# NikolaZubic/2dimageto3dmodel

Hardware: NVIDIA H100
Metric: render+loss+GAN images/sec (cfg3: cfg2 render+loss at batch 32 + conv-GAN 256x256 G/D iteration, 1 G : 2 D, Adam) (higher is better)
Workload: dtype tf32 (convs) / f32

## Files before the change

2dimageto3dmodel_b200/b3d/conv.py:

```python
import ctypes

import torch

from . import B3DError, check, dev, last_variant, lib, ptr, stream_ptr
from .bank import LayerWeights

VARIANT_LOG = None


def _conv_call(fn, *args):
    rc = fn(*args)
    if VARIANT_LOG is not None and rc == 0:
        VARIANT_LOG.extend(v for v in last_variant().split(";") if v)
    return rc


def _ints(v):
    return (ctypes.c_int * len(v))(*v)


def _pad_last(t, mult):
    c = t.shape[-1]
    return t if c % mult == 0 else torch.nn.functional.pad(t, (0, mult - c % mult))

# ... 204 lines not shown
        N, H, W, _ = x.shape
        gy = dev(gy, "grad_output")
        st = stream_ptr(gy)
        gb = None
        want_gb = has_bias and ctx.needs_input_grad[2]
        g_pitch = 0
        link_out = ctx.link_out
        if link_out is not None and link_out.done:
            link_out.done = False
            if tuple(gy.shape) != tuple(y.shape):
                raise B3DError("conv2d: chained gradient has the wrong shape")
            g_pitch = y.shape[2]
            gb = link_out.gb if want_gb else None
            link_out.gb = None
            gy = gy[:, :, pad_out:y.shape[2] - pad_out]
        elif pad_out:
            _, Ho, OW, _ = y.shape
            masked = torch.empty(N, Ho, OW - 2 * pad_out, Cout, device=gy.device, dtype=torch.float32)
            gb = torch.zeros(Cout, device=gy.device, dtype=torch.float32) if want_gb else None
            check(lib.b3d_pad_leaky_bias_bwd(ptr(gy), ptr(y), ptr(masked), ptr(gb), N * Ho, OW - 2 * pad_out, Cout, pad_out,
                                             pad_mode, float(leaky), st))
            gy = masked
        elif leaky != 1.0:
            masked = torch.empty_like(gy)
            check(lib.b3d_leaky_bwd(ptr(gy), ptr(y), ptr(masked), gy.numel(), float(leaky), st))
            gy = masked
        if gb is None and want_gb:
            gb = gy.sum(dim=(0, 1, 2))
        gx = gw = None
        if ctx.needs_input_grad[0]:
            link_in = ctx.link_in
            sums = torch.zeros(2 * Cin, device=gy.device, dtype=torch.float64) if link_in is not None and link_in.want_gb else None
            gx = _dgrad(gy, lw.wd if lw.wd is not None else _d_layout(lw.wf.detach()), (gy.shape[1] if fold_raw else H, W), kh,
                        kw, pad_y, stride, x_crop, g_pitch, x if link_in is not None else None,
                        link_in.slope if link_in is not None else 1.0, sums)
            if link_in is not None:
                check(lib.b3d_wrap_x_bwd_inplace(ptr(gx), N * H, W - 2 * link_in.pad, Cin, link_in.pad, link_in.mode, st))
                link_in.gb = sums[:Cin].float() if sums is not None else None
                link_in.done = True
            if fold_raw:
                graw = torch.empty(N, H, W, Cx, device=gy.device, dtype=torch.float32)
                check(lib.b3d_fold_rows_bwd(ptr(gx), ptr(graw), N, H, W, Cx, lw.kh, fold_pad, Cin, st))
                gx = graw
            elif Cx != Cin:
                gx = gx[..., :Cx]
        if ctx.needs_input_grad[1]:
            if fold_raw:
                gw = _wgrad(gy, x, kh, kw, fold_pad, stride, x_crop, lw.df, g_pitch, fold_raw, Cin)
            else:
                gw = _wgrad(gy, x, kh, kw, pad_y, stride, x_crop, lw.df, g_pitch)
            if lw.df is None:
                gw = gw[:, :lw.Cin]
        return gx, gw, gb, None, None, None, None, None, None, None, None, None, None, None, None


def fold_kh_weight(weight, cpad=0):
    Cout, Cin, kh, kw = weight.shape
    w = weight.permute(0, 2, 1, 3).reshape(Cout, kh * Cin, 1, kw)
    return torch.nn.functional.pad(w, (0, 0, 0, 0, 0, cpad)) if cpad else w


def conv2d(x_nchw, weight, bias=None, pad_y=0, stride=1, leaky=1.0, pad_out=0, pad_mode=1, x_crop=0):
    x = x_nchw.permute(0, 2, 3, 1)
    Cout, Cin, kh, kw = weight.shape
    if stride == 1 and kh > 1 and Cin * kh <= 64:
        from .ew import fold_rows
        cpad = (-kh * Cin) % 32
        x = fold_rows(x, kh, pad_y, kh * Cin + cpad)
        weight = fold_kh_weight(weight, cpad)
        Cout, Cin, kh, kw = weight.shape
        pad_y = 0
    lw = LayerWeights(dict(Cout=Cout, Cin=Cin, kh=kh, kw=kw, fold=0, Cinp=-(-Cin // 32) * 32, Coutp=-(-Cout // 32) * 32,
                           Tp=kh * kw))
    lw.wf = _pad_last(taps_layout(weight.detach()), 32)
    y = _Conv.apply(x, weight, bias, lw, int(pad_y), int(stride), float(leaky), int(pad_out), int(pad_mode), int(x_crop))
    return y.permute(0, 3, 1, 2)


def conv2d_banked(x_nchw, lw, pad_y=0, stride=1, leaky=1.0, pad_out=0, pad_mode=1, x_crop=0, stats=None, link_in=None, link_out=None):
    x = x_nchw.permute(0, 2, 3, 1)
    fold_raw, fold_fwd = 0, False
    if lw.fold:
        Wout = x.shape[2] - lw.kw + 1
        if (lw.Cin == 8 and lw.kw == 5 and lw.Cinp == 64 and stride == 1 and not x_crop and Wout % 128 == 0
                and x.shape[0] * x.shape[1] * (Wout // 128) >= 2 * torch.cuda.get_device_properties(x.device).multi_processor_count):
            fold_raw = lw.kh
            fold_fwd = torch.is_grad_enabled() and lw.wf.requires_grad
        else:
            from .ew import fold_rows
            x = fold_rows(x, lw.kh, pad_y, lw.Cinp)
    y = _Conv.apply(x, lw.wf, lw.bias, lw, int(pad_y), int(stride), float(leaky), int(pad_out), int(pad_mode), int(x_crop), stats,
                    fold_raw, link_in, link_out, fold_fwd)
    return y.permute(0, 3, 1, 2)
```

2dimageto3dmodel_b200/csrc/b3d_core.cu:

```cuda
#include <atomic>
#include <stdarg.h>
#include <string.h>

#include "b3d_common.cuh"

namespace b3d {
static thread_local char g_err[512] = "";
static thread_local char g_variant[256] = "";
static std::atomic<uint64_t> g_launches{0};

void set_error(const char* fmt, ...) {
    va_list ap;
    va_start(ap, fmt);
    vsnprintf(g_err, sizeof(g_err), fmt, ap);
    va_end(ap);
}
void clear_variant() { g_variant[0] = 0; }
void add_variant(const char* fmt, ...) {
    size_t n = strlen(g_variant);
    if (n + 2 >= sizeof(g_variant)) return;
    if (n) g_variant[n++] = ';';
    va_list ap;
    va_start(ap, fmt);
    vsnprintf(g_variant + n, sizeof(g_variant) - n, fmt, ap);
    va_end(ap);
}
void count_launch(int n) { g_launches.fetch_add((uint64_t)n, std::memory_order_relaxed); }
}

extern "C" {
const char* b3d_last_error(void) { return b3d::g_err; }
const char* b3d_last_variant(void) { return b3d::g_variant; }
int b3d_version(void) { return 420; }
uint64_t b3d_launch_count(void) { return b3d::g_launches.load(std::memory_order_relaxed); }
}
```

2dimageto3dmodel_b200/csrc/tc_conv.cu:

```cuda
#include "tc_common.cuh"

namespace {

constexpr int BM = 128;
constexpr int BK = 32;
constexpr int MMA_K = 8;
constexpr int MAX_TAPS = 25;
constexpr int NTHREADS = 384;

struct ConvParams {
    int N, Hout, Wout, Cout;
    int BW, BH, BI;
    int tiles_x, tiles_y;
    int xbase;
    int ntaps, kslices;
    int sy, sx;
    int dy[MAX_TAPS], dx[MAX_TAPS];
    int wtap[MAX_TAPS];
    int OH, OW, OC, osy, osx;
    float leaky;
    double* stats;
    int fold;
    int fold_y0;
    int mask;
    float mslope;
    int stats_sum;
    int ncls;
    int cooy[4], coox[4];
    uint32_t esn, esy, esx;
    int dx0, shift[5];
};

constexpr int MASK_BYTES = BM * BK * 4;
template <int BN, int STAGES, int KW>
struct CSmem {
    static constexpr int WIN_BYTES = (BM + KW - 1) * BK * 4;
    static constexpr int A_BYTES = (WIN_BYTES + 1023) / 1024 * 1024;
    static constexpr int B_BYTES = KW * BN * BK * 4;
    static constexpr int STAGE_BYTES = A_BYTES + B_BYTES;
    static constexpr int TX_BYTES = WIN_BYTES + B_BYTES;
    static constexpr int TOTAL = STAGES * STAGE_BYTES + 1024  + 256 ;
    static_assert(A_BYTES >= MASK_BYTES, "a mask chunk does not fit the A region of a stage");
};

__device__ __forceinline__ uint32_t mask_offset(int px, int ch) { return px * 128 + ((((ch >> 2) ^ px) & 7) << 4) + (ch & 3) * 4; }

template <int BN>
constexpr bool kCoop = BN > 128;
template <int BN>
constexpr int kBlocks = (kCoop<BN> ? BN / 2 : BN) / 64;
template <int BN>
constexpr int kEmptyArrivals = kCoop<BN> ? 8 : 4;
template <int BN>
constexpr int kLeaderArrivals = kEmptyArrivals<BN> / (kCoop<BN> ? 2 : 1);
static_assert(kLeaderArrivals<64> == 4 && kLeaderArrivals<128> == 4 && kLeaderArrivals<256> == 4,
              "a leader stands for the 4 warps of its warpgroup");
template <int BN>
constexpr int kMaskGroup = kCoop<BN> ? 4 : 2;
__host__ __device__ constexpr int mask_chunk_channel(int i, int G) { return 128 * ((i % G) / 2) + 64 * (i / G) + 32 * (i % 2); }

template <int BN, int STAGES, int KW, bool FOLD>
__device__ __forceinline__ void mainloop(float (&acc)[kBlocks<BN>][BM / 2], unsigned char* base, uint64_t* full, uint64_t* empty,
                                         int KI, uint32_t& git, uint32_t& phase, int cb, bool leader, const int* shift) {
    constexpr int A_BYTES = CSmem<BN, STAGES, KW>::A_BYTES, STAGE = CSmem<BN, STAGES, KW>::STAGE_BYTES;
    for (int it = 0; it < KI; ++it, ++git) {
        const int s = git % STAGES;
        tc::mbar_wait(full + s, (phase >> s) & 1);
        phase ^= 1u << s;
        const uint32_t a = tc::smem_u32(base + s * STAGE), b = a + A_BYTES + cb * 128;
        tc::wgmma_fence();
#pragma unroll
        for (int t = 0; t < KW; ++t) {
            const uint32_t shifted = a + (KW > 1 ? shift[t] * 128 : 0);
#pragma unroll
            for (int k = 0; k < BK / MMA_K; ++k) {
                const uint32_t acc_flag = (it | t | k) ? 1u : 0u;
                const uint64_t dp = FOLD ? tc::desc_k32(a + k * (BM * 32)) : tc::desc_k128(shifted + k * MMA_K * 4);
#pragma unroll
                for (int m = 0; m < kBlocks<BN>; ++m)
                    tc::Wgmma<BM>::mma(acc[m], tc::desc_k128(b + t * (BN * 128) + m * (64 * 128) + k * MMA_K * 4), dp, acc_flag);
            }
        }
        tc::wgmma_commit();
        tc::wgmma_wait<1>();
        if (it > 0 && leader) tc::mbar_arrive(empty + (git - 1) % STAGES, kLeaderArrivals<BN>);
    }
    tc::wgmma_wait<0>();
    if (KI > 0 && leader) tc::mbar_arrive(empty + (git - 1) % STAGES, kLeaderArrivals<BN>);
}

struct TileAt {
    int n0, y0, x0;
    size_t base;
    int lbw, lbwh;
};
__device__ __forceinline__ void tile_origin(const ConvParams& p, TileAt& t, int tile, int cls) {
    t.x0 = p.xbase + (tile % p.tiles_x) * p.BW;
    t.y0 = (tile / p.tiles_x) % p.tiles_y * p.BH;
    t.n0 = tile / (p.tiles_x * p.tiles_y) * p.BI;
    t.base = (((size_t)t.n0 * p.OH + (size_t)(p.osy * t.y0 + p.cooy[cls])) * p.OW + (size_t)(p.osx * t.x0 + p.coox[cls])) * p.OC;
}
__device__ __forceinline__ bool tile_pixel(const ConvParams& p, const TileAt& t, int px, uint32_t& rel) {
    const int bi = px >> t.lbwh, by = (px >> t.lbw) & (p.BH - 1), bx = px & (p.BW - 1);
    rel = bi * p.esn + by * p.esy + bx * p.esx;
    return t.n0 + bi < p.N && t.y0 + by < p.Hout && t.x0 + bx < p.Wout;
}

template <int G, int STAGES>
__device__ __forceinline__ void mask_bits(uint32_t (&neg)[2], uint32_t mstage, int cw, int lane, uint64_t* empty, uint32_t g0) {
    int q;
    asm volatile("mov.u32 %0, 0;" : "=r"(q));
    q += 2 * (lane & 3);
    uint32_t mb[4];
#pragma unroll
    for (int i = 0; i < 4; ++i) mb[i] = mstage + mask_offset(q + (i & 1), (cw + 8 * (i >> 1)) & 31);
#pragma unroll
    for (int hf = 0; hf < 2; ++hf) {
        uint32_t bits = 0;
#pragma unroll
        for (int j = 0; j < BM / 16; ++j)
#pragma unroll
            for (int i = 0; i < 4; ++i) bits |= (tc::lds_f32(mb[i] + 1024 * (j + 8 * hf)) >= 0.f ? 0u : 1u) << (4 * j + i);
        neg[hf] = bits;
    }
    __syncwarp();
    if (lane == 0)
#pragma unroll
        for (int i = 0; i < G; ++i) tc::mbar_arrive(empty + (g0 + i) % STAGES);
}

template <bool MASKED>
__device__ __forceinline__ void epilogue_block(const float (&acc)[BM / 2], const uint32_t (&neg)[2], const ConvParams& p, const TileAt& t,
                                               const float* bias, float* out, int c0, int cw, int lane) {
    bool cok[2];
    float bv[2], sum[2] = {0.f, 0.f}, sq[2] = {0.f, 0.f};
#pragma unroll
    for (int e = 0; e < 2; ++e) {
        cok[e] = c0 + cw + 8 * e < p.Cout;
        bv[e] = bias && cok[e] ? __ldg(bias + c0 + cw + 8 * e) : 0.f;
    }
    float* out0 = out + t.base + c0 + cw;
    int q;
    asm volatile("mov.u32 %0, 0;" : "=r"(q));
    q += 2 * (lane & 3);
#pragma unroll
    for (int j = 0; j < BM / 8; ++j) {
#pragma unroll
        for (int e1 = 0; e1 < 2; ++e1) {
            uint32_t rel;
            const bool valid = tile_pixel(p, t, 8 * j + q + e1, rel);
#pragma unroll
            for (int e2 = 0; e2 < 2; ++e2) {
                float v = acc[4 * j + 2 * e2 + e1];
                if constexpr (MASKED) v *= (neg[j / 8] >> (4 * (j % 8) + 2 * e2 + e1)) & 1u ? p.mslope : 1.f;
                v = valid ? v : 0.f;
                sum[e2] += v;
                sq[e2] += v * v;
                if (valid && cok[e2]) {
                    const float o = v + bv[e2];
                    out0[rel + 8 * e2] = o >= 0.f ? o : o * p.leaky;
                }
            }
        }
    }
    if (p.stats) {
#pragma unroll
        for (int e = 0; e < 2; ++e) {
            sum[e] += __shfl_xor_sync(0xffffffffu, sum[e], 1);
            sum[e] += __shfl_xor_sync(0xffffffffu, sum[e], 2);
            sq[e] += __shfl_xor_sync(0xffffffffu, sq[e], 1);
            sq[e] += __shfl_xor_sync(0xffffffffu, sq[e], 2);
            if ((lane & 3) == 0 && cok[e]) {
                atomicAdd(p.stats + c0 + cw + 8 * e, (double)sum[e]);
                if (!p.stats_sum) atomicAdd(p.stats + p.Cout + c0 + cw + 8 * e, (double)sq[e]);
            }
        }
    }
}

constexpr int PRODUCER_REGS = 24, CONSUMER_REGS = 240;

template <int BN, int STAGES, int KW>
__global__ void __launch_bounds__(NTHREADS, 1)
conv_wgmma_kernel(const __grid_constant__ CUtensorMap tmap_x, const __grid_constant__ CUtensorMap tmap_w,
                  const __grid_constant__ CUtensorMap tmap_m, const ConvParams p, const float* __restrict__ bias,
                  float* __restrict__ out, int tiles, int work_items) {
    using S = CSmem<BN, STAGES, KW>;
    constexpr bool COOP = kCoop<BN>;
    constexpr int OWNERS = COOP ? 1 : 2;
    constexpr int G = kMaskGroup<BN>;
    static_assert(G <= STAGES, "the mask stages of one block do not fit the ring");
    extern __shared__ unsigned char smem_raw[];
    unsigned char* base = reinterpret_cast<unsigned char*>((reinterpret_cast<uintptr_t>(smem_raw) + 1023) & ~uintptr_t(1023));
    uint64_t* full = reinterpret_cast<uint64_t*>(base + STAGES * S::STAGE_BYTES);
    uint64_t* empty = full + OWNERS * STAGES;
    static_assert((OWNERS + 1) * STAGES * 8 <= 256, "barriers do not fit their area");
    if (threadIdx.x == 0) {
        tc::tma_prefetch_desc(&tmap_x);
        tc::tma_prefetch_desc(&tmap_w);
        if (p.mask) tc::tma_prefetch_desc(&tmap_m);
        for (int s = 0; s < STAGES; ++s) {
            for (int o = 0; o < OWNERS; ++o) tc::mbar_init(full + o * STAGES + s, 1);
            tc::mbar_init(empty + s, kEmptyArrivals<BN>);
        }
        tc::fence_barrier_init();
    }
    __syncthreads();
    const int KI = p.ntaps / KW * p.kslices;
    const int MS = p.mask ? BN / 32 : 0;
    const int wg = threadIdx.x >> 7;

    if (wg == 0) {
        tc::setmaxnreg_dec<PRODUCER_REGS>();
        if (threadIdx.x == 0) {
            uint32_t git = 0;
            for (int w = blockIdx.x, k = 0; w < work_items; w += gridDim.x, ++k) {
                uint64_t* fb = full + (COOP ? 0 : (k & 1) * STAGES);
                const int cls = w % p.ncls, wq = w / p.ncls, tb = cls * p.ntaps;
                int t = wq % tiles;
                const int c0 = (wq / tiles) * BN;
                const int x0 = p.xbase + (t % p.tiles_x) * p.BW;
                t /= p.tiles_x;
                const int y0 = (t % p.tiles_y) * p.BH, n0 = (t / p.tiles_y) * p.BI;
                for (int it = 0; it < KI; ++it, ++git) {
                    const int s = git % STAGES;
                    tc::mbar_wait(empty + s, ((git / STAGES) & 1) ^ 1);
                    const int tap = it / p.kslices * KW, ks = it % p.kslices;
                    unsigned char* a = base + s * S::STAGE_BYTES;
                    tc::mbar_arrive_expect_tx(fb + s, S::TX_BYTES);
                    if (KW > 1)
                        tc::tma_load_4d(a, &tmap_x, fb + s, ks * BK, x0 + p.dx0, y0 + p.dy[tb + tap], n0);
                    else if (p.fold)
                        tc::tma_load_4d(a, &tmap_x, fb + s, 0, x0 + p.dx[tb + tap], y0 + p.fold_y0 + 4 * ks, n0);
                    else
                        tc::tma_load_4d(a, &tmap_x, fb + s, ks * BK, p.sx * x0 + p.dx[tb + tap], p.sy * y0 + p.dy[tb + tap], n0);
                    tc::tma_load_3d(a + S::A_BYTES, &tmap_w, fb + s, ks * BK, c0, p.wtap[tb + tap]);
                }
                const int mx = p.osx * x0 + p.coox[cls], my = p.osy * y0 + p.cooy[cls];
                for (int m = 0; m < MS; ++m, ++git) {
                    const int s = git % STAGES;
                    tc::mbar_wait(empty + s, ((git / STAGES) & 1) ^ 1);
                    tc::mbar_arrive_expect_tx(fb + s, MASK_BYTES);
                    tc::tma_load_4d(base + s * S::STAGE_BYTES, &tmap_m, fb + s, c0 + mask_chunk_channel(m, G), mx, my, n0);
                }
            }
        }
        return;
    }
    tc::setmaxnreg_inc<CONSUMER_REGS>();

    const int h = wg - 1, tid = threadIdx.x & 127, lane = tid & 31;
    float acc[kBlocks<BN>][BM / 2];
#pragma unroll
    for (int m = 0; m < kBlocks<BN>; ++m)
#pragma unroll
        for (int i = 0; i < BM / 2; ++i) acc[m][i] = 0.f;
    uint32_t git = 0, phase = 0;
    const uint32_t ring = tc::smem_u32(base);
    TileAt at;
    at.lbw = __ffs(p.BW) - 1;
    at.lbwh = at.lbw + __ffs(p.BH) - 1;
    uint64_t* fb = full + (COOP ? 0 : h * STAGES);
    const int cb = COOP ? 128 * h : 0;
    const int cw = (tid >> 5) * 16 + (lane >> 2);
    const int mine = (COOP ? 2 * h : 0) + (tid >> 6);
    for (int k = COOP ? 0 : h;; k += COOP ? 1 : 2) {
        const int w = blockIdx.x + k * gridDim.x;
        if (w >= work_items) break;
        git = (uint32_t)k * (KI + MS);
        const int wq = w / p.ncls, tile = wq % tiles, c0 = (wq / tiles) * BN + cb;
        tile_origin(p, at, tile, w % p.ncls);
        if (KW == 1 && p.fold) mainloop<BN, STAGES, KW, true>(acc, base, fb, empty, KI, git, phase, cb, tid == 0, p.shift);
        else mainloop<BN, STAGES, KW, false>(acc, base, fb, empty, KI, git, phase, cb, tid == 0, p.shift);
        uint32_t neg[kBlocks<BN>][2] = {};
        if (p.mask) {
#pragma unroll
            for (int m = 0; m < kBlocks<BN>; ++m, git += G) {
                uint32_t mstage = 0;
#pragma unroll
                for (int i = 0; i < G; ++i) {
                    const int s = (git + i) % STAGES;
                    tc::mbar_wait(fb + s, (phase >> s) & 1);
                    phase ^= 1u << s;
                    if (i == mine) mstage = ring + s * S::STAGE_BYTES;
                }
                mask_bits<G, STAGES>(neg[m], mstage, cw, lane, empty, git);
            }
        }
#pragma unroll
        for (int m = 0; m < kBlocks<BN>; ++m) {
            if (p.mask) epilogue_block<true>(acc[m], neg[m], p, at, bias, out, c0 + 64 * m, cw, lane);
            else epilogue_block<false>(acc[m], neg[m], p, at, bias, out, c0 + 64 * m, cw, lane);
        }
    }
}

struct WgradParams {
    int N, Hout, Wout, Cout, Cin;
    int BWk, BHk;
    int kx, ky;
    int kh, kw, pad_y, st;
    int xoff;
    int splits;
    int tapmajor;
    int tstep;
};

template <int BN, int STAGES, int NRAW, int T>
struct WSmem {
    static constexpr int DY_BYTES = BM * BK * 4;
    static constexpr int STAGE_BYTES = T * BN * BK * 4;
    static constexpr int WROWS = T == 1 ? 32 : 36;
    static constexpr int RAW_X = (BN / 32) * WROWS * 128;
    static constexpr int RAW_BYTES = (DY_BYTES + RAW_X + 1023) / 1024 * 1024;
    static constexpr int TOTAL = STAGES * STAGE_BYTES + NRAW * RAW_BYTES + 1024 + 256;
};

__host__ __device__ constexpr int wgrad_row_co(int m) { return (m & 35) | ((m & 8) >> 1) | ((m & 16) >> 1) | ((m & 4) << 2); }

__host__ __device__ constexpr int dy_tile_offset(int co, int px) {
    return (co >> 5) * 4096 + px * 128 + ((((co >> 2) & 7) ^ (px & 7)) << 4) + (co & 3) * 4;
}

__host__ __device__ constexpr int xt_chunk(int i) { return (((i & 7) >> 1) ^ ((i >> 4) & 3)) | (((i >> 3) & 1) << 2); }
__host__ __device__ constexpr int xt_src_offset(int i, int px, int wrows) { return ((i >> 6) * wrows + px) * 128 + (i & 7) * 16; }
__host__ __device__ constexpr int xt_dst_offset(int i, int j) {
    return ((i >> 6) * 32 + 4 * (i & 7) + j) * 128 + ((xt_chunk(i) ^ ((4 * (i & 7) + j) & 7)) << 4);
}
template <int BN, int T, int WROWS>
__device__ __forceinline__ void wgrad_transpose(uint32_t src, uint32_t dst, int tid) {
    constexpr int NT = 2 * BN / 128;
    float4 v[NT][T + 3];
#pragma unroll
    for (int n = 0; n < NT; ++n)
#pragma unroll
        for (int u = 0; u < T + 3; ++u) v[n][u] = tc::lds_f32x4(src + xt_src_offset(tid + 128 * n, 4 * xt_chunk(tid + 128 * n) + u, WROWS));
#pragma unroll
    for (int n = 0; n < NT; ++n) {
        const int i = tid + 128 * n;
#pragma unroll
        for (int t = 0; t < T; ++t) {
            const uint32_t d = dst + t * (BN * 128);
            const float4* w = v[n] + t;
            tc::sts_f32x4(d + xt_dst_offset(i, 0), w[0].x, w[1].x, w[2].x, w[3].x);
            tc::sts_f32x4(d + xt_dst_offset(i, 1), w[0].y, w[1].y, w[2].y, w[3].y);
            tc::sts_f32x4(d + xt_dst_offset(i, 2), w[0].z, w[1].z, w[2].z, w[3].z);
            tc::sts_f32x4(d + xt_dst_offset(i, 3), w[0].w, w[1].w, w[2].w, w[3].w);
        }
    }
}

template <int N, int T, int STAGES, int NRAW, int RAW_BYTES, int STAGE_BYTES>
__device__ __forceinline__ void wgrad_consume(float (&acc)[T][N / 2], uint32_t raw_s, uint32_t stage_s, uint64_t* full,
                                              uint64_t* empty, uint64_t* rawfull, uint64_t* rawempty, const int (&aoff)[4],
                                              int first, int step, int KI, int tid, bool zero_first) {
    using Frag = uint32_t[BK / MMA_K][4];
// ... 303 lines not shown
                    atomicAdd(dw + ((size_t)co * p.Cin + ci + 1) * STEM_KW + t, v1);
                }
            }
        }
    }
}

int wgrad_splits(int base_ctas, long long ktotal) {
    constexpr long long FIXED = 16;
    const long long sms = tc::num_sms();
    long long smax = ktotal / 8;
    if (smax > 8 * sms) smax = 8 * sms;
    int best = 1;
    long long best_cost = -1;
    for (long long s = 1; s <= smax; ++s) {
        const long long cost = (base_ctas * s + sms - 1) / sms * ((ktotal + s - 1) / s + FIXED);
        if (best_cost < 0 || cost < best_cost) { best = (int)s; best_cost = cost; }
    }
    return best;
}

template <int BN, int STAGES, int KW = 1>
int launch_conv(const CUtensorMap& mx, const CUtensorMap& mw, const CUtensorMap& mm, const ConvParams& p, const float* bias, float* out,
                int tiles, cudaStream_t st) {
    using S = CSmem<BN, STAGES, KW>;
    static_assert(S::TOTAL <= 227 * 1024, "conv pipeline does not fit shared memory");
    B3D_CUDA_OK(cudaFuncSetAttribute(conv_wgmma_kernel<BN, STAGES, KW>, cudaFuncAttributeMaxDynamicSharedMemorySize, S::TOTAL));
    const int work = tiles * b3d::ceil_div(p.Cout, BN) * p.ncls;
    const int sms = tc::num_sms();
    conv_wgmma_kernel<BN, STAGES, KW><<<work < sms ? work : sms, NTHREADS, S::TOTAL, st>>>(mx, mw, mm, p, bias, out, tiles, work);
    B3D_LAUNCH_OK();
    if (KW > 1) b3d::add_variant("conv_wgmma_rowwin<%d,%d,%d>", BN, KW, STAGES);
    else b3d::add_variant("conv_wgmma<%d,%d>", BN, STAGES);
    return B3D_OK;
}

template <int BN>
int launch_rowwin(int kw, const CUtensorMap& mx, const CUtensorMap& mw, const CUtensorMap& mm, const ConvParams& p, const float* bias,
                  float* out, int tiles, cudaStream_t st) {
    if (kw == 2) return launch_conv<BN, BN == 64 ? 5 : 4, 2>(mx, mw, mm, p, bias, out, tiles, st);
    if (kw == 3) return launch_conv<BN, BN == 64 ? 4 : 3, 3>(mx, mw, mm, p, bias, out, tiles, st);
    return launch_conv<BN, BN == 64 ? 3 : 2, 5>(mx, mw, mm, p, bias, out, tiles, st);
}

int pow2_floor(int v) {
    int p = 1;
    while (p * 2 <= v) p *= 2;
    return p;
}

}

extern "C" {

int b3d_conv2d_tf32(const float* x, const float* wt, const float* bias, float* out, int N, int H, int W, int Cin,
                    int Hout, int Wout, int Cout, int ntaps, const int* dy, const int* dx, int sy, int sx, int OH,
                    int OW, int OC, int osy, int osx, int ooy, int oox, float leaky, const int* wtap,
                    int wtaps_total, double* stats, int fold_kh, int fold_pad, const b3d_conv_opts* opts, void* stream) {
    B3D_REQUIRE(N > 0 && H > 0 && W > 0 && Hout > 0 && Wout > 0 && Cout > 0, B3D_EINVAL, "b3d_conv2d_tf32: bad sizes");
    B3D_REQUIRE(Cin > 0 && Cin % BK == 0, B3D_EINVAL, "b3d_conv2d_tf32: Cin=%d must be a multiple of %d", Cin, BK);
    B3D_REQUIRE(ntaps >= 1 && ntaps <= MAX_TAPS && dy && dx, B3D_EINVAL, "b3d_conv2d_tf32: bad taps");
    B3D_REQUIRE(x && wt && out, B3D_EINVAL, "b3d_conv2d_tf32: null pointer");
    B3D_REQUIRE(sy >= 1 && sy <= 2 && sx >= 1 && sx <= 2, B3D_EINVAL, "b3d_conv2d_tf32: stride must be 1 or 2");
    if (!wtap) wtaps_total = ntaps;
    B3D_REQUIRE(wtaps_total >= ntaps || wtap, B3D_EINVAL, "b3d_conv2d_tf32: bad weight tap count");
    for (int t = 0; wtap && t < ntaps; ++t)
        B3D_REQUIRE(wtap[t] >= 0 && wtap[t] < wtaps_total, B3D_EINVAL, "b3d_conv2d_tf32: weight tap %d out of range", wtap[t]);
    B3D_CHECK_ALIGNED(x);
    B3D_CHECK_ALIGNED(wt);
    b3d::clear_variant();

    const float* mask = opts ? opts->mask : nullptr;
    const float mslope = opts ? opts->mask_slope : 1.f;
    B3D_REQUIRE(!mask || (reinterpret_cast<uintptr_t>(mask) % 16 == 0 && OC % 4 == 0), B3D_EINVAL,
                "b3d_conv2d_tf32: the mask needs a 16-byte aligned base and OC %% 4 == 0 (OC=%d)", OC);
    const int stats_sum = (opts && opts->stats_sum_only) ? 1 : 0;
    const int xpitch = (opts && opts->x_row_pitch) ? opts->x_row_pitch : W;
    const int ncls = (opts && opts->nclass > 1) ? opts->nclass : 1;
    B3D_REQUIRE(ncls <= 4 && ntaps % ncls == 0 && (ncls == 1 || (sy == 1 && sx == 1 && fold_kh == 0)), B3D_EINVAL,
                "b3d_conv2d_tf32: nclass=%d needs <= 4 equal tap groups of a stride-1 launch", ncls);
    const int tpc = ntaps / ncls;
    int cooy[4] = {ooy, ooy, ooy, ooy}, coox[4] = {oox, oox, oox, oox};
    for (int c = 0; c < ncls && ncls > 1; ++c) { cooy[c] = opts->class_ooy[c]; coox[c] = opts->class_oox[c]; }
    B3D_REQUIRE(xpitch >= W && (fold_kh == 0 || xpitch == W), B3D_EINVAL, "b3d_conv2d_tf32: x_row_pitch=%d must be >= W=%d (and absent with the on-the-fly fold)", xpitch, W);
    if (fold_kh > 0) {
        B3D_REQUIRE(fold_kh <= 8 && Cin == 32 * ((8 * fold_kh + 31) / 32) && sy == 1 && sx == 1 && !wtap && Wout % BM == 0,
                    B3D_EINVAL, "b3d_conv2d_tf32: on-the-fly fold needs 8 input channels, stride 1 and Wout %% 128 == 0 (Wout=%d)", Wout);
    }
    B3D_REQUIRE(!stats || mask || (osy == 1 && osx == 1), B3D_EINVAL, "b3d_conv2d_tf32: statistics need a dense output");
    const bool bn256 = Cout % 256 == 0 && (long long)N * Hout * Wout / BM * (Cout / 256) * ncls >= tc::num_sms();
    const int BN = bn256 ? 256 : Cout > 64 ? 128 : 64;
    cudaStream_t st = (cudaStream_t)stream;
    CUtensorMap mw;
    {
        const uint64_t dims[3] = {(uint64_t)Cin, (uint64_t)Cout, (uint64_t)wtaps_total};
        const uint64_t strides[2] = {(uint64_t)Cin * 4, (uint64_t)Cout * Cin * 4};
        const uint32_t box[3] = {(uint32_t)BK, (uint32_t)BN, 1};
        if (int rc = tc::make_tmap_f32(&mw, wt, 3, dims, strides, box)) return rc;
    }

    int g_kw = 0, g_step = 1, g_wstep = 1;
    if (sy == 1 && sx == 1 && fold_kh == 0) {
        int kw_ = 1;
        while (kw_ < tpc && dy[kw_] == dy[0]) ++kw_;
        const int step = kw_ > 1 ? dx[1] - dx[0] : 1;
        const int wstep = (wtap && kw_ > 1) ? wtap[1] - wtap[0] : 1;
        bool grid_ok = tpc % kw_ == 0 && (kw_ == 2 || kw_ == 3 || kw_ == 5) && (step == 1 || step == -1) && wstep >= 1 && wstep <= 2 &&
                       (ncls == 1 || wtap != nullptr);
        for (int t = 0; grid_ok && t < ntaps; ++t) {
            const int tc_ = t % tpc, t0 = t - tc_;
            grid_ok = dy[t] == dy[t0 + (tc_ / kw_) * kw_] && dx[t] == dx[0] + (tc_ % kw_) * step;
            if (wtap) grid_ok = grid_ok && wtap[t] == wtap[t0 + (tc_ / kw_) * kw_] + (tc_ % kw_) * wstep;
        }
        if (grid_ok && BN <= 128) { g_kw = kw_; g_step = step; g_wstep = wstep; }
    }

    auto run = [&](int xlo, int xhi) -> int {
        const int wspan = xhi - xlo;
        ConvParams p{};
        p.N = N; p.Hout = Hout; p.Wout = xhi; p.Cout = Cout; p.xbase = xlo;
        p.BW = pow2_floor(wspan < BM ? wspan : BM);
        p.BH = pow2_floor(Hout < BM / p.BW ? Hout : BM / p.BW);
        p.BI = BM / (p.BW * p.BH);
        p.tiles_x = b3d::ceil_div(wspan, p.BW);
        p.tiles_y = b3d::ceil_div(Hout, p.BH);
        const int tiles = p.tiles_x * p.tiles_y * b3d::ceil_div(N, p.BI);
        p.ntaps = tpc; p.kslices = Cin / BK; p.sy = sy; p.sx = sx; p.ncls = ncls;
        for (int t = 0; t < ntaps; ++t) { p.dy[t] = dy[t]; p.dx[t] = dx[t]; p.wtap[t] = wtap ? wtap[t] : t; }
        for (int c = 0; c < 4; ++c) { p.cooy[c] = cooy[c]; p.coox[c] = coox[c]; }
        p.OH = OH; p.OW = OW; p.OC = OC; p.osy = osy; p.osx = osx;
        p.leaky = leaky;
        p.stats = stats;
        p.mask = mask != nullptr; p.mslope = mslope; p.stats_sum = stats_sum;
        p.fold = fold_kh; p.fold_y0 = -fold_pad;
        {
            const unsigned long long esn = p.BI > 1 ? (unsigned long long)OH * OW * OC : 0, esy = p.BH > 1 ? (unsigned long long)osy * OW * OC : 0,
                                     esx = (unsigned long long)osx * OC;
            B3D_REQUIRE((p.BI - 1) * esn + (p.BH - 1) * esy + (p.BW - 1) * esx + OC < (1ull << 32), B3D_EINVAL,
                        "b3d_conv2d_tf32: a %d x %d x %d pixel tile spans more than 2^32 elements of the output", p.BI, p.BH, p.BW);
            p.esn = (uint32_t)esn; p.esy = (uint32_t)esy; p.esx = (uint32_t)esx;
        }
        CUtensorMap mm{};
        if (mask) {
            const uint64_t dims[4] = {(uint64_t)OC, (uint64_t)OW, (uint64_t)OH, (uint64_t)N};
            const uint64_t strides[3] = {(uint64_t)OC * 4, (uint64_t)OW * OC * 4, (uint64_t)OH * OW * OC * 4};
            const uint32_t box[4] = {(uint32_t)BK, (uint32_t)(osx * (p.BW - 1) + 1), (uint32_t)(osy * (p.BH - 1) + 1), (uint32_t)p.BI};
            const uint32_t es[4] = {1, (uint32_t)osx, (uint32_t)osy, 1};
            if (int rc = tc::make_tmap_f32(&mm, mask, 4, dims, strides, box, es)) return rc;
        }
        CUtensorMap mx;
        if (g_kw && wspan >= BM) {
            p.dx0 = g_step > 0 ? dx[0] : dx[g_kw - 1];
            for (int t = 0; t < g_kw; ++t) p.shift[t] = dx[t] - p.dx0;
            const uint64_t dims[4] = {(uint64_t)Cin, (uint64_t)W, (uint64_t)H, (uint64_t)N};
            const uint64_t strides[3] = {(uint64_t)Cin * 4, (uint64_t)xpitch * Cin * 4, (uint64_t)H * xpitch * Cin * 4};
            const uint32_t box[4] = {(uint32_t)BK, (uint32_t)(BM + g_kw - 1), 1, 1};
            if (int rc = tc::make_tmap_f32(&mx, x, 4, dims, strides, box)) return rc;
            CUtensorMap mwr;
            const uint64_t wdims[3] = {(uint64_t)Cin, (uint64_t)Cout, (uint64_t)wtaps_total};
            const uint64_t wstrides[2] = {(uint64_t)Cin * 4, (uint64_t)Cout * Cin * 4};
            const uint32_t wbox[3] = {(uint32_t)BK, (uint32_t)BN, (uint32_t)((g_kw - 1) * g_wstep + 1)};
            const uint32_t wes[3] = {1, 1, (uint32_t)g_wstep};
            if (int rc = tc::make_tmap_f32(&mwr, wt, 3, wdims, wstrides, wbox, wes)) return rc;
            return BN == 128 ? launch_rowwin<128>(g_kw, mx, mwr, mm, p, bias, out, tiles, st)
                             : launch_rowwin<64>(g_kw, mx, mwr, mm, p, bias, out, tiles, st);
        }
        if (fold_kh > 0) {
            B3D_REQUIRE(p.BH == 1 && p.BI == 1, B3D_EINVAL, "b3d_conv2d_tf32: on-the-fly fold needs one-row tiles");
            const uint64_t dims[4] = {8, (uint64_t)W, (uint64_t)H, (uint64_t)N};
            const uint64_t strides[3] = {32, (uint64_t)W * 32, (uint64_t)H * W * 32};
            const uint32_t box[4] = {8, (uint32_t)p.BW, 4, 1};
            if (int rc = tc::make_tmap_f32(&mx, x, 4, dims, strides, box, nullptr, CU_TENSOR_MAP_SWIZZLE_32B)) return rc;
        } else {
            const uint64_t dims[4] = {(uint64_t)Cin, (uint64_t)W, (uint64_t)H, (uint64_t)N};
            const uint64_t strides[3] = {(uint64_t)Cin * 4, (uint64_t)xpitch * Cin * 4, (uint64_t)H * xpitch * Cin * 4};
            const uint32_t box[4] = {(uint32_t)BK, (uint32_t)(sx * (p.BW - 1) + 1), (uint32_t)(sy * (p.BH - 1) + 1), (uint32_t)p.BI};
            const uint32_t es[4] = {1, (uint32_t)sx, (uint32_t)sy, 1};
            if (int rc = tc::make_tmap_f32(&mx, x, 4, dims, strides, box, es)) return rc;
        }
        if (BN == 256) return launch_conv<256, 4>(mx, mw, mm, p, bias, out, tiles, st);
        if (BN == 128) return launch_conv<128, 6>(mx, mw, mm, p, bias, out, tiles, st);
        return launch_conv<64, 8>(mx, mw, mm, p, bias, out, tiles, st);
    };
    const int bw_full = pow2_floor(Wout < BM ? Wout : BM);
    const int rem = Wout % bw_full;
    if (rem != 0 && rem * 8 <= bw_full && Wout > bw_full) {
        const int rc = run(0, Wout - rem);
        return rc ? rc : run(Wout - rem, Wout);
    }
    return run(0, Wout);
}

int b3d_conv2d_wgrad_tf32(const float* dy, const float* x, float* dw, int N, int H, int W, int Cin, int Hout, int Wout,
                          int Cout, int kh, int kw, int pad_y, int stride, int x_off, int tap_major, int fold_kh, int dy_row_pitch,
                          void* stream) {
    B3D_REQUIRE(N > 0 && Cin > 0 && Cout > 0 && H > 0 && W > 0 && Hout > 0 && Wout > 0, B3D_EINVAL,
                "b3d_conv2d_wgrad_tf32: bad sizes");
    B3D_REQUIRE(kh * kw <= MAX_TAPS && (stride == 1 || stride == 2) && x_off >= 0, B3D_EINVAL, "b3d_conv2d_wgrad_tf32: bad kernel/stride");
    B3D_REQUIRE(dy && x && dw, B3D_EINVAL, "b3d_conv2d_wgrad_tf32: null pointer");
    B3D_REQUIRE(Cin % 32 == 0 && Cout % 32 == 0, B3D_EINVAL,
                "b3d_conv2d_wgrad_tf32: Cin=%d and Cout=%d must be multiples of 32 (pad the channels with zeros)", Cin, Cout);
    B3D_CHECK_ALIGNED(dy);
    B3D_CHECK_ALIGNED(x);
    b3d::clear_variant();
    if (tap_major) B3D_CHECK_ALIGNED(dw);
    WgradParams p{};
    p.N = N; p.Hout = Hout; p.Wout = Wout; p.Cout = Cout; p.Cin = Cin;
    const uint64_t dpitch = dy_row_pitch > 0 ? dy_row_pitch : Wout;
    B3D_REQUIRE(dpitch >= (uint64_t)Wout, B3D_EINVAL, "b3d_conv2d_wgrad_tf32: dy_row_pitch=%d must be >= Wout=%d", dy_row_pitch, Wout);
    cudaStream_t st = (cudaStream_t)stream;
    if (fold_kh > 0) {
        B3D_REQUIRE(fold_kh > 4 && fold_kh <= 8 && Cin == 64 && kh == 1 && kw == STEM_KW && stride == 1 && x_off == 0 &&
                        Cout % 64 == 0 && W == Wout + STEM_KW - 1 && Hout == H + 2 * pad_y - fold_kh + 1,
                    B3D_EINVAL, "b3d_conv2d_wgrad_tf32: the raw-input stem weight gradient needs 4 < fold_kh <= 8 rows folded into "
                    "64 channels, a 1x5 stride-1 filter, Cout %% 64 == 0 and the x padding in the input");
        p.BWk = BK; p.BHk = 1;
        p.kx = b3d::ceil_div(Wout, BK);
        p.ky = Hout;
        p.kh = 1; p.kw = kw; p.pad_y = pad_y; p.st = 1; p.tapmajor = tap_major ? 1 : 0;
        p.splits = wgrad_splits(Cout / 64, (long long)N * p.kx * p.ky);
        CUtensorMap mdy, mx;
        {
            const uint64_t dims[5] = {32, (uint64_t)Wout, (uint64_t)Hout, (uint64_t)N, (uint64_t)Cout / 32};
            const uint64_t strides[4] = {(uint64_t)Cout * 4, dpitch * Cout * 4, (uint64_t)Hout * dpitch * Cout * 4, 128};
            const uint32_t box[5] = {32, (uint32_t)BK, 1, 1, 2};
            if (int rc = tc::make_tmap_f32(&mdy, dy, 5, dims, strides, box)) return rc;
        }
        {
            const uint64_t dims[4] = {8, (uint64_t)W, (uint64_t)H, (uint64_t)N};
            const uint64_t strides[3] = {32, (uint64_t)W * 32, (uint64_t)H * W * 32};
            const uint32_t box[4] = {8, (uint32_t)StemSmem::WPX, (uint32_t)fold_kh, 1};
            if (int rc = tc::make_tmap_f32(&mx, x, 4, dims, strides, box, nullptr, CU_TENSOR_MAP_SWIZZLE_NONE)) return rc;
        }
        B3D_CUDA_OK(cudaFuncSetAttribute(wgrad_stem_kernel, cudaFuncAttributeMaxDynamicSharedMemorySize, StemSmem::TOTAL));
        wgrad_stem_kernel<<<dim3(Cout / 64, p.splits), NTHREADS, StemSmem::TOTAL, st>>>(mdy, mx, p, fold_kh, dw);
        B3D_LAUNCH_OK();
        b3d::add_variant("wgrad_stem<%d,%d,%d>", STEM_KW, STEM_STAGES, STEM_NRAW);
        return B3D_OK;
    }
    p.BWk = pow2_floor(Wout < BK ? Wout : BK);
    p.BHk = BK / p.BWk;
    p.kx = b3d::ceil_div(Wout, p.BWk);
    p.ky = b3d::ceil_div(Hout, p.BHk);
    p.kh = kh; p.kw = kw; p.pad_y = pad_y; p.st = stride; p.xoff = x_off; p.tapmajor = tap_major ? 1 : 0;
    const int BN = Cin > 64 ? 128 : 64;
    int T = 1;
    p.tstep = 1;
    if (Wout >= BK) {
        if (stride == 1 && kw == 3 && BN == 64) T = 3;
        if (stride == 2 && kw == 4) { T = 2; p.tstep = 2; }
    }
    const int base_ctas = b3d::ceil_div(Cout, BM) * b3d::ceil_div(Cin, BN) * kh * (kw / T);
    const long long ktotal = (long long)N * p.kx * p.ky;
    const int splits = wgrad_splits(base_ctas, ktotal);
    p.splits = splits;
// ... 25 lines not shown
```

Measured before the change: 1440.

## Add dedicated stem-conv path with resident weights and shared row window

Replaces the on-the-fly fold path for the 5x5, 8-channel stem convolution with a specialised producer/consumer pair. All 25 tap weights are loaded once into shared memory per CTA. Each work item then loads a single 5-row by 132-pixel input window and issues 25 k=8 wgmma calls over shifted views of that window, instead of streaming folded slices and weights per K-step. This cuts redundant input and weight TMA traffic for the stem layer. In exchange the fold path is restricted to Cout=64, kh=5 and contiguous taps, and each tile waits on its wgmma before the epilogue, with no overlap between them.

```diff
diff --git a/2dimageto3dmodel_b200/b3d/conv.py b/2dimageto3dmodel_b200/b3d/conv.py
--- a/2dimageto3dmodel_b200/b3d/conv.py
+++ b/2dimageto3dmodel_b200/b3d/conv.py
@@ -310,7 +310,8 @@
     fold_raw, fold_fwd = 0, False
     if lw.fold:
         Wout = x.shape[2] - lw.kw + 1
-        if (lw.Cin == 8 and lw.kw == 5 and lw.Cinp == 64 and stride == 1 and not x_crop and Wout % 128 == 0
+        if (lw.Cin == 8 and lw.kh == 5 and lw.kw == 5 and lw.Cinp == 64 and lw.Cout == 64 and stride == 1 and not x_crop
+                and Wout % 128 == 0
                 and x.shape[0] * x.shape[1] * (Wout // 128) >= 2 * torch.cuda.get_device_properties(x.device).multi_processor_count):
             fold_raw = lw.kh
             fold_fwd = torch.is_grad_enabled() and lw.wf.requires_grad
diff --git a/2dimageto3dmodel_b200/csrc/b3d_core.cu b/2dimageto3dmodel_b200/csrc/b3d_core.cu
--- a/2dimageto3dmodel_b200/csrc/b3d_core.cu
+++ b/2dimageto3dmodel_b200/csrc/b3d_core.cu
@@ -31,6 +31,6 @@
 extern "C" {
 const char* b3d_last_error(void) { return b3d::g_err; }
 const char* b3d_last_variant(void) { return b3d::g_variant; }
-int b3d_version(void) { return 420; }
+int b3d_version(void) { return 430; }
 uint64_t b3d_launch_count(void) { return b3d::g_launches.load(std::memory_order_relaxed); }
 }
diff --git a/2dimageto3dmodel_b200/csrc/tc_conv.cu b/2dimageto3dmodel_b200/csrc/tc_conv.cu
--- a/2dimageto3dmodel_b200/csrc/tc_conv.cu
+++ b/2dimageto3dmodel_b200/csrc/tc_conv.cu
@@ -59,7 +59,7 @@
 constexpr int kMaskGroup = kCoop<BN> ? 4 : 2;
 __host__ __device__ constexpr int mask_chunk_channel(int i, int G) { return 128 * ((i % G) / 2) + 64 * (i / G) + 32 * (i % 2); }
 
-template <int BN, int STAGES, int KW, bool FOLD>
+template <int BN, int STAGES, int KW>
 __device__ __forceinline__ void mainloop(float (&acc)[kBlocks<BN>][BM / 2], unsigned char* base, uint64_t* full, uint64_t* empty,
                                          int KI, uint32_t& git, uint32_t& phase, int cb, bool leader, const int* shift) {
     constexpr int A_BYTES = CSmem<BN, STAGES, KW>::A_BYTES, STAGE = CSmem<BN, STAGES, KW>::STAGE_BYTES;
@@ -75,7 +75,7 @@
 #pragma unroll
             for (int k = 0; k < BK / MMA_K; ++k) {
                 const uint32_t acc_flag = (it | t | k) ? 1u : 0u;
-                const uint64_t dp = FOLD ? tc::desc_k32(a + k * (BM * 32)) : tc::desc_k128(shifted + k * MMA_K * 4);
+                const uint64_t dp = tc::desc_k128(shifted + k * MMA_K * 4);
 #pragma unroll
                 for (int m = 0; m < kBlocks<BN>; ++m)
                     tc::Wgmma<BM>::mma(acc[m], tc::desc_k128(b + t * (BN * 128) + m * (64 * 128) + k * MMA_K * 4), dp, acc_flag);
@@ -175,6 +175,63 @@
                 if (!p.stats_sum) atomicAdd(p.stats + p.Cout + c0 + cw + 8 * e, (double)sq[e]);
             }
         }
+    }
+}
+
+constexpr int SW_KH = 5, SW_KW = 5, SW_PX = BM + SW_KW - 1;
+constexpr int SW_TAP_BYTES = 64 * 32;
+constexpr int SW_W_BYTES = SW_KH * SW_KW * SW_TAP_BYTES;
+constexpr int SW_WIN_BYTES = SW_KH * SW_PX * 32;
+constexpr int SW_STAGE_BYTES = (SW_WIN_BYTES + 1023) / 1024 * 1024;
+constexpr int SW_STAGES = (8 * CSmem<64, 8, 1>::STAGE_BYTES - SW_W_BYTES) / SW_STAGE_BYTES;
+static_assert(SW_STAGES >= 2 && SW_STAGES <= 8, "the stem window ring does not fit the ring of conv_wgmma<64,8>");
+
+template <int STAGES>
+__device__ __forceinline__ void stem_producer(const CUtensorMap* tmap_x, const CUtensorMap* tmap_w, const ConvParams& p,
+                                              unsigned char* base, uint64_t* full, uint64_t* empty, uint64_t* wbar, int work_items) {
+    tc::mbar_arrive_expect_tx(wbar, SW_W_BYTES);
+    for (int t = 0; t < SW_KH * SW_KW; ++t)
+        tc::tma_load_3d(base + t * SW_TAP_BYTES, tmap_w, wbar, 8 * (t / SW_KW), 0, t % SW_KW);
+    for (int w = blockIdx.x, k = 0; w < work_items; w += gridDim.x, ++k) {
+        const int s = k % SW_STAGES, t = w / p.tiles_x;
+        uint64_t* fb = full + (k & 1) * STAGES;
+        tc::mbar_wait(empty + s, ((k / SW_STAGES) & 1) ^ 1);
+        tc::mbar_arrive_expect_tx(fb + s, SW_WIN_BYTES);
+        tc::tma_load_4d(base + SW_W_BYTES + s * SW_STAGE_BYTES, tmap_x, fb + s, 0, (w % p.tiles_x) * BM + p.dx0,
+                        t % p.tiles_y + p.fold_y0, t / p.tiles_y);
+    }
+}
+
+__device__ __forceinline__ void stem_consumer(const ConvParams& p, unsigned char* base, uint64_t* fb, uint64_t* empty, uint64_t* wbar,
+                                              const float* bias, float* out, int work_items, int h, int tid) {
+    float acc[BM / 2];
+#pragma unroll
+    for (int i = 0; i < BM / 2; ++i) acc[i] = 0.f;
+    const int lane = tid & 31, cw = (tid >> 5) * 16 + (lane >> 2);
+    const uint32_t wts = tc::smem_u32(base), ring = wts + SW_W_BYTES, neg[2] = {0u, 0u};
+    TileAt at;
+    at.lbw = at.lbwh = 7;
+    uint32_t phase = 0;
+    tc::mbar_wait(wbar, 0);
+    for (int k = h;; k += 2) {
+        const int w = blockIdx.x + k * gridDim.x;
+        if (w >= work_items) break;
+        tile_origin(p, at, w, 0);
+        const int s = k % SW_STAGES;
+        tc::mbar_wait(fb + s, (phase >> s) & 1);
+        phase ^= 1u << s;
+        const uint32_t win = ring + s * SW_STAGE_BYTES;
+        tc::wgmma_fence();
+#pragma unroll
+        for (int c = 0; c < SW_KW; ++c)
+#pragma unroll
+            for (int r = 0; r < SW_KH; ++r)
+                tc::Wgmma<BM>::mma(acc, tc::desc_k32(wts + (r * SW_KW + c) * SW_TAP_BYTES), tc::desc_k32(win + (r * SW_PX + c) * 32),
+                                   (r | c) ? 1u : 0u);
+        tc::wgmma_commit();
+        tc::wgmma_wait<0>();
+        if (tid == 0) tc::mbar_arrive(empty + s, kLeaderArrivals<64>);
+        epilogue_block<false>(acc, neg, p, at, bias, out, 0, cw, lane);
     }
 }
 
@@ -194,7 +251,9 @@
     unsigned char* base = reinterpret_cast<unsigned char*>((reinterpret_cast<uintptr_t>(smem_raw) + 1023) & ~uintptr_t(1023));
     uint64_t* full = reinterpret_cast<uint64_t*>(base + STAGES * S::STAGE_BYTES);
     uint64_t* empty = full + OWNERS * STAGES;
-    static_assert((OWNERS + 1) * STAGES * 8 <= 256, "barriers do not fit their area");
+    uint64_t* wbar = empty + STAGES;
+    static_assert((OWNERS + 1) * STAGES * 8 + 8 <= 256, "barriers do not fit their area");
+    constexpr bool STEM = BN == 64 && STAGES == 8 && KW == 1;
     if (threadIdx.x == 0) {
         tc::tma_prefetch_desc(&tmap_x);
         tc::tma_prefetch_desc(&tmap_w);
@@ -203,6 +262,7 @@
             for (int o = 0; o < OWNERS; ++o) tc::mbar_init(full + o * STAGES + s, 1);
             tc::mbar_init(empty + s, kEmptyArrivals<BN>);
         }
+        if (STEM && p.fold) tc::mbar_init(wbar, 1);
         tc::fence_barrier_init();
     }
     __syncthreads();
@@ -212,6 +272,12 @@
 
     if (wg == 0) {
         tc::setmaxnreg_dec<PRODUCER_REGS>();
+        if constexpr (STEM) {
+            if (p.fold) {
+                if (threadIdx.x == 0) stem_producer<STAGES>(&tmap_x, &tmap_w, p, base, full, empty, wbar, work_items);
+                return;
+            }
+        }
         if (threadIdx.x == 0) {
             uint32_t git = 0;
             for (int w = blockIdx.x, k = 0; w < work_items; w += gridDim.x, ++k) {
@@ -230,8 +296,6 @@
                     tc::mbar_arrive_expect_tx(fb + s, S::TX_BYTES);
                     if (KW > 1)
                         tc::tma_load_4d(a, &tmap_x, fb + s, ks * BK, x0 + p.dx0, y0 + p.dy[tb + tap], n0);
-                    else if (p.fold)
-                        tc::tma_load_4d(a, &tmap_x, fb + s, 0, x0 + p.dx[tb + tap], y0 + p.fold_y0 + 4 * ks, n0);
                     else
                         tc::tma_load_4d(a, &tmap_x, fb + s, ks * BK, p.sx * x0 + p.dx[tb + tap], p.sy * y0 + p.dy[tb + tap], n0);
                     tc::tma_load_3d(a + S::A_BYTES, &tmap_w, fb + s, ks * BK, c0, p.wtap[tb + tap]);
@@ -250,6 +314,12 @@
     tc::setmaxnreg_inc<CONSUMER_REGS>();
 
     const int h = wg - 1, tid = threadIdx.x & 127, lane = tid & 31;
+    if constexpr (STEM) {
+        if (p.fold) {
+            stem_consumer(p, base, full + h * STAGES, empty, wbar, bias, out, work_items, h, tid);
+            return;
+        }
+    }
     float acc[kBlocks<BN>][BM / 2];
 #pragma unroll
     for (int m = 0; m < kBlocks<BN>; ++m)
@@ -270,8 +340,7 @@
         git = (uint32_t)k * (KI + MS);
         const int wq = w / p.ncls, tile = wq % tiles, c0 = (wq / tiles) * BN + cb;
         tile_origin(p, at, tile, w % p.ncls);
-        if (KW == 1 && p.fold) mainloop<BN, STAGES, KW, true>(acc, base, fb, empty, KI, git, phase, cb, tid == 0, p.shift);
-        else mainloop<BN, STAGES, KW, false>(acc, base, fb, empty, KI, git, phase, cb, tid == 0, p.shift);
+        mainloop<BN, STAGES, KW>(acc, base, fb, empty, KI, git, phase, cb, tid == 0, p.shift);
         uint32_t neg[kBlocks<BN>][2] = {};
         if (p.mask) {
 #pragma unroll
@@ -741,10 +810,14 @@
     const int tpc = ntaps / ncls;
     int cooy[4] = {ooy, ooy, ooy, ooy}, coox[4] = {oox, oox, oox, oox};
     for (int c = 0; c < ncls && ncls > 1; ++c) { cooy[c] = opts->class_ooy[c]; coox[c] = opts->class_oox[c]; }
-    B3D_REQUIRE(xpitch >= W && (fold_kh == 0 || xpitch == W), B3D_EINVAL, "b3d_conv2d_tf32: x_row_pitch=%d must be >= W=%d (and absent with the on-the-fly fold)", xpitch, W);
+    B3D_REQUIRE(xpitch >= W && (fold_kh == 0 || xpitch == W), B3D_EINVAL, "b3d_conv2d_tf32: x_row_pitch=%d must be >= W=%d (and absent with the stem window)", xpitch, W);
     if (fold_kh > 0) {
-        B3D_REQUIRE(fold_kh <= 8 && Cin == 32 * ((8 * fold_kh + 31) / 32) && sy == 1 && sx == 1 && !wtap && Wout % BM == 0,
-                    B3D_EINVAL, "b3d_conv2d_tf32: on-the-fly fold needs 8 input channels, stride 1 and Wout %% 128 == 0 (Wout=%d)", Wout);
+        bool taps_ok = ntaps == SW_KW && dx[0] >= 0 && dx[0] + Wout + SW_KW - 1 <= W;
+        for (int t = 1; t < ntaps && taps_ok; ++t) taps_ok = dx[t] == dx[0] + t;
+        B3D_REQUIRE(fold_kh == SW_KH && taps_ok && Cin == 64 && Cout == 64 && sy == 1 && sx == 1 && !wtap && !mask && ncls == 1 &&
+                        Wout % BM == 0,
+                    B3D_EINVAL, "b3d_conv2d_tf32: the stem window needs a 5 x 5 filter on 8 input channels folded into 64, 64 output "
+                    "channels, stride 1, the x padding in the input and Wout %% 128 == 0 (Wout=%d, Cout=%d)", Wout, Cout);
     }
     B3D_REQUIRE(!stats || mask || (osy == 1 && osx == 1), B3D_EINVAL, "b3d_conv2d_tf32: statistics need a dense output");
     const bool bn256 = Cout % 256 == 0 && (long long)N * Hout * Wout / BM * (Cout / 256) * ncls >= tc::num_sms();
@@ -825,11 +898,17 @@
                              : launch_rowwin<64>(g_kw, mx, mwr, mm, p, bias, out, tiles, st);
         }
         if (fold_kh > 0) {
-            B3D_REQUIRE(p.BH == 1 && p.BI == 1, B3D_EINVAL, "b3d_conv2d_tf32: on-the-fly fold needs one-row tiles");
+            p.dx0 = dx[0];
             const uint64_t dims[4] = {8, (uint64_t)W, (uint64_t)H, (uint64_t)N};
             const uint64_t strides[3] = {32, (uint64_t)W * 32, (uint64_t)H * W * 32};
-            const uint32_t box[4] = {8, (uint32_t)p.BW, 4, 1};
+            const uint32_t box[4] = {8, (uint32_t)SW_PX, (uint32_t)SW_KH, 1};
             if (int rc = tc::make_tmap_f32(&mx, x, 4, dims, strides, box, nullptr, CU_TENSOR_MAP_SWIZZLE_32B)) return rc;
+            CUtensorMap mws;
+            const uint64_t wdims[3] = {(uint64_t)Cin, (uint64_t)Cout, (uint64_t)ntaps};
+            const uint64_t wstrides[2] = {(uint64_t)Cin * 4, (uint64_t)Cout * Cin * 4};
+            const uint32_t wbox[3] = {8, 64, 1};
+            if (int rc = tc::make_tmap_f32(&mws, wt, 3, wdims, wstrides, wbox, nullptr, CU_TENSOR_MAP_SWIZZLE_32B)) return rc;
+            return launch_conv<64, 8>(mx, mws, mm, p, bias, out, tiles, st);
         } else {
             const uint64_t dims[4] = {(uint64_t)Cin, (uint64_t)W, (uint64_t)H, (uint64_t)N};
             const uint64_t strides[3] = {(uint64_t)Cin * 4, (uint64_t)xpitch * Cin * 4, (uint64_t)H * xpitch * Cin * 4};
```

After: 1459 (median of 6 runs). +1.3%, better.
